# MiloszKrajewski/K4os.Compression.LZ4

Hardware: AMD Instinct MI355X
Metric: GiB/s encode+decode on batched 64 KiB blocks; bit-exact vs C# ref (higher is better)
Workload: dtype u8

## Files before the change

k4os/compression/lz4_amd/csrc/k4lz4_capi.hip:

```cpp
#include <hip/hip_runtime.h>
#include <stdint.h>
#include <stdio.h>
#include <stdlib.h>
#include <string.h>
#include <algorithm>
#include <atomic>
#include <memory>
#include <new>
#include <condition_variable>
#include <functional>
#include <mutex>
#include <string>
#include <thread>
#include <chrono>
#include <vector>

#include "../../../../include/k4lz4.h"
#include "k4lz4_decode.hpp"
#include "k4lz4_encode_fast.hpp"
#include "k4lz4_parse.hpp"
#include "k4lz4_pickle.hpp"
#include "k4lz4_segments.hpp"
#include "k4lz4_encode_hc.hpp"
#include "k4lz4_fast_chain.hpp"
#include "k4lz4_frame.hpp"
#include "k4lz4_frame_read.hpp"
#include "k4lz4_legacy.hpp"
#include "k4lz4_frame_write.hpp"
#include "k4lz4_frame_reader.hpp"
#include "k4lz4_frame_feed.hpp"
#include "k4lz4_legacy_stream.hpp"
#include "k4lz4_legacy_feed.hpp"
#include "k4lz4_chain_decoder.hpp"
#include "k4lz4_xxh32.hpp"
#include "k4lz4_selftest.hpp"

constexpr int MAX_PARTS = 8;

struct k4lz4_ctx {
    int device = -1;
    std::string error;
    hipStream_t stream = nullptr;
    int accel = 1;
    unsigned long long *prof = nullptr;
    bool prof_pair = false;
    bool prof_stamp = false;
    uint8_t *d_src = nullptr; size_t d_src_cap = 0;
    uint8_t *d_dst = nullptr; size_t d_dst_cap = 0;
    uint8_t *d_meta = nullptr; size_t d_meta_cap = 0;
    uint8_t *h_stage = nullptr; size_t h_stage_cap = 0;
    uint8_t *d_sched = nullptr; size_t d_sched_cap = 0;
    int cu_count = 256;
    uint8_t *d_dict = nullptr; size_t d_dict_cap = 0;
    uint8_t *d_gtab = nullptr; size_t d_gtab_cap = 0;
    hipStream_t aux = nullptr;
    hipStream_t aux2 = nullptr;
    hipEvent_t ev_join2 = nullptr;
    uint8_t *d_seg = nullptr; size_t d_seg_cap = 0;
    uint8_t *d_seg_first = nullptr; size_t d_seg_first_cap = 0;
    bool use_segments = true;
    uint32_t seg_min = 1024u << 10, seg_target = 640u << 10, seg_warm = 384u << 10;
    uint32_t seg_target_max = 1408u << 10;
    uint32_t seg_spin_max = 0;
    uint32_t seg_div = 3500;
    hipEvent_t ev_fork = nullptr, ev_join = nullptr;
    uint8_t *d_hc_hash = nullptr; size_t d_hc_hash_cap = 0;
    uint8_t *d_hc_work = nullptr; size_t d_hc_work_cap = 0;
    uint8_t *d_hc_meta = nullptr; size_t d_hc_meta_cap = 0;
    uint8_t *d_pk_meta = nullptr; size_t d_pk_meta_cap = 0;
    int pickle_split_min = 512;
    hipEvent_t ev_busy = nullptr;
    hipStream_t last_stream = nullptr;
    bool busy = false;
    uint64_t hc_res_total = 0; uint32_t hc_res_longest = 0;
    uint8_t *h_in[2] = {nullptr, nullptr}; size_t h_in_cap[2] = {0, 0};
    uint8_t *h_out[2] = {nullptr, nullptr}; size_t h_out_cap[2] = {0, 0};
    hipEvent_t ev_in[2] = {nullptr, nullptr}, ev_out[2] = {nullptr, nullptr};
    uint8_t *d_pack = nullptr; size_t d_pack_cap = 0;
    hipStream_t copyq = nullptr;
    hipStream_t dlq = nullptr;
    hipEvent_t ev_up[MAX_PARTS] = {}, ev_len[MAX_PARTS] = {};
    uint8_t *h_len = nullptr; size_t h_len_cap = 0;
    struct Pool *pool = nullptr, *pool_dl = nullptr;
    bool pool_failed = false, pool_dl_failed = false;
    int stage_threads = 7;
    uint32_t *d_pace = nullptr;
    uint32_t *d_status = nullptr;
    int split_pct = -1;
    bool no_pair = false;
    int direct_span_pct = 200;
    bool no_direct = false;
    int lds_floor_per_cu = 8;
    int cost_pct = 48;
    int dec_parts = 4, dec_parts_direct = 8;
    int hop2_max_per_cu = 12;
    bool hc_cand_lds = true;
    int hc_cand_dynlds = 0;
    int hc_segs = 0;
    bool hc_chain_parts = true;
    int hc_mem_pct = 33;
    int pace_min_per_cu = 6;
    bool use_pace = true;
    bool prof_gtab = false;
    uint8_t *d_parse = nullptr; size_t d_parse_cap = 0;
    bool use_parse = true;
    bool parse_queue = false;
    bool hc_records = true;
    bool parse_seg = true;
    bool parse_big = true;
    bool parse_persist = true;
    bool parse_inline_emit = true;
    bool parse_migrate = true;
    bool parse_pcost = false;
    int parse_waves = 16;
    bool trace = false;
    std::vector<uint8_t> h_chain;
    uint8_t *d_chain = nullptr; size_t d_chain_cap = 0;
    hipEvent_t ev_chain = nullptr;
    uint8_t *d_fr = nullptr; size_t d_fr_cap = 0;
    uint8_t *d_fb = nullptr; size_t d_fb_cap = 0;
    uint8_t *d_lg = nullptr; size_t d_lg_cap = 0;
    uint8_t *d_frd = nullptr; size_t d_frd_cap = 0;
    uint8_t *d_lgr = nullptr; size_t d_lgr_cap = 0;
    uint8_t *d_lga = nullptr; size_t d_lga_cap = 0;
    std::vector<uint8_t> h_fw;
    uint8_t *d_fw = nullptr; size_t d_fw_cap = 0;
    hipEvent_t ev_fw = nullptr;
};

struct Pool {
    std::vector<std::thread> workers;
    std::mutex m;
    std::condition_variable cv_work, cv_done;
    std::function<void(int)> job;
    int parts = 0, next = 0, pending = 0;
    unsigned long long gen = 0;
    bool stop = false;
    explicit Pool(int nthreads)
    {
        for (int t = 0; t < nthreads; t++) workers.emplace_back([this] { run(); });
    }
    ~Pool()
    {
        { std::lock_guard<std::mutex> g(m); stop = true; }
        cv_work.notify_all();
// ... 8 lines not shown
            const int i = next++;
            lk.unlock();
            job(i);
            lk.lock();
            if (--pending == 0) cv_done.notify_all();
        }
    }
    void parallel(int nparts, const std::function<void(int)> &f)
    {
        if (nparts <= 1 || workers.empty()) { for (int i = 0; i < nparts; i++) f(i); return; }
        std::unique_lock<std::mutex> lk(m);
        job = f; parts = nparts; next = 0; pending = nparts; gen++;
        cv_work.notify_all();
        while (next < parts) {
            const int i = next++;
            lk.unlock();
            f(i);
            lk.lock();
            if (--pending == 0) cv_done.notify_all();
        }
        cv_done.wait(lk, [this] { return pending == 0; });
        parts = 0;
    }
};

namespace {

thread_local std::string tl_error;
thread_local int tl_status = K4LZ4_OK;

std::mutex g_err_mu;
int fail(k4lz4_ctx *ctx, int code, const std::string &msg)
{
    if (ctx) { std::lock_guard<std::mutex> g(g_err_mu); ctx->error = msg; }
    tl_error = msg;
    return code;
}

int hip_fail(k4lz4_ctx *ctx, hipError_t e, const char *what)
{
    char buf[256];
    snprintf(buf, sizeof buf, "%s: %s", what, hipGetErrorString(e));
    (void)hipGetLastError();
    return fail(ctx, K4LZ4_E_HIP, buf);
}

#define K4_HIP(ctx, call)                                                   \
    do {                                                                    \
        hipError_t e_ = (call);                                             \
        if (e_ != hipSuccess) return hip_fail(ctx, e_, #call);              \
    } while (0)

enum Kind { KIND_ENCODE, KIND_DECODE, KIND_PICKLE, KIND_UNPICKLE, KIND_WRAP };
enum Envelope { ENV_NONE, ENV_PICKLE, ENV_WRAP };
constexpr int FLAG_SEGMENTS_OK = 1 << 20;

std::atomic<int> g_enforce32{0};

int check_level(k4lz4_ctx *ctx, int level)
{
    (void)ctx; (void)level;
    return K4LZ4_OK;
}

int grow(k4lz4_ctx *ctx, uint8_t **p, size_t *cap, size_t need, bool pinned);

int take_device_status(k4lz4_ctx *ctx)
// ... 238 lines not shown
            const int64_t cnt = std::min<int64_t>(chunk_max, n - first);
            const size_t need_meta = (size_t)cnt * 16 + 64;
            if (need_meta > ctx->d_pk_meta_cap) K4_HIP(ctx, hipStreamSynchronize(stream));
            int rc = grow(ctx, &ctx->d_pk_meta, &ctx->d_pk_meta_cap, need_meta, false);
            if (rc != K4LZ4_OK) return rc;
            uint64_t *d_encoff = (uint64_t *)ctx->d_pk_meta;
            int32_t *d_enccap = (int32_t *)(d_encoff + cnt);
            int32_t *d_enclen = d_enccap + cnt;
            k4::BatchArgs a{};
            a.src = src; a.srcOff = srcOff + first; a.srcLen = srcLen + first; a.dst = dst; a.dstOff = dstOff + first;
            a.dstCap = dstCap + first; a.outLen = outLen + first; a.n = cnt; a.level = level; a.accel = 1;
            a.flags = flags | (g_enforce32.load(std::memory_order_relaxed) ? K4LZ4_FLAG_X32 : 0);
            const int seg_ok = kind == KIND_PICKLE || may_cut ? FLAG_SEGMENTS_OK : 0;
            if (kind == KIND_PICKLE) hipLaunchKernelGGL(k4::k4_pickle_prep_kernel, dim3((unsigned)((cnt + 255) / 256)), dim3(256), 0, stream, a, d_encoff, d_enccap);
            else hipLaunchKernelGGL(k4::k4_wrap_prep_kernel, dim3((unsigned)((cnt + 255) / 256)), dim3(256), 0, stream, a, d_encoff, d_enccap);
            rc = launch_inner(ctx, KIND_ENCODE, src, srcOff + first, srcLen + first, dst, d_encoff, d_enccap, d_enclen, cnt, level,
                              (flags & (K4LZ4_FLAG_NO_REORDER | K4LZ4_FLAG_X32)) | K4LZ4_FLAG_RAW_RETURN | seg_ok, stream, nullptr, hostLen ? hostLen + first : nullptr);
            if (rc != K4LZ4_OK) return rc;
            if (kind == KIND_PICKLE) hipLaunchKernelGGL(k4::k4_pickle_finish_kernel, dim3((unsigned)((cnt + k4::PICKLE_FINISH_WAVES_PER_WG - 1) / k4::PICKLE_FINISH_WAVES_PER_WG)), dim3(64 * k4::PICKLE_FINISH_WAVES_PER_WG), 0, stream, a, d_enclen);
            else hipLaunchKernelGGL(k4::k4_wrap_finish_kernel, dim3((unsigned)((cnt + k4::WRAP_FINISH_WAVES_PER_WG - 1) / k4::WRAP_FINISH_WAVES_PER_WG)), dim3(64 * k4::WRAP_FINISH_WAVES_PER_WG), 0, stream, a, d_enclen);
            K4_HIP(ctx, hipGetLastError());
        }
        return K4LZ4_OK;
    }
    const bool reorder = n > 1 &&
                         (encode_like ? !(flags & K4LZ4_FLAG_NO_REORDER)
                                      : ((flags & K4LZ4_FLAG_REORDER) != 0 ||
                                         (kind == KIND_UNPICKLE && n > 64 && !(flags & K4LZ4_FLAG_NO_REORDER))));
    uint32_t *d_cost = nullptr, *d_order = nullptr, *d_hist = nullptr;
    if (reorder) {
        const size_t cnt_max = (size_t)std::min<int64_t>(chunk_max, n);
        const size_t hist_words = std::max<size_t>(2 * (size_t)k4::PCOST_BUCKETS, 2 * (size_t)k4::COST_BUCKETS + 16);
        const size_t need = cnt_max * 8 + hist_words * 4 + 64;
        if (need > ctx->d_sched_cap) K4_HIP(ctx, hipStreamSynchronize(stream));
        int rc = grow(ctx, &ctx->d_sched, &ctx->d_sched_cap, need, false);
        if (rc != K4LZ4_OK) return rc;
        d_hist = (uint32_t *)ctx->d_sched;
        d_cost = d_hist + hist_words;
        d_order = d_cost + cnt_max;
    }
    for (int64_t first = 0; first < n; first += chunk_max) {
        const int64_t cnt = std::min<int64_t>(chunk_max, n - first);
        k4::BatchArgs a{};
        a.src = src; a.srcOff = srcOff + first; a.srcLen = srcLen + first;
        a.dst = dst; a.dstOff = dstOff + first; a.dstCap = dstCap + first;
        a.outLen = outLen + first; a.n = cnt; a.level = level; a.accel = ctx->accel;
        a.flags = flags | (g_enforce32.load(std::memory_order_relaxed) ? K4LZ4_FLAG_X32 : 0);
        const bool hop2 = cnt <= (int64_t)ctx->hop2_max_per_cu * (int64_t)ctx->cu_count;
        a.prof = ctx->prof ? ctx->prof + k4::PROF_STRIDE * first : nullptr;
        a.status = ctx->d_status;
        if (((kind == KIND_ENCODE && !parse_path) || (K4_DEC_PACE && (kind == KIND_DECODE || kind == KIND_UNPICKLE))) && ctx->use_pace && ctx->d_pace && cnt > (int64_t)ctx->pace_min_per_cu * (int64_t)ctx->cu_count) {
            a.pace = ctx->d_pace;
            K4_HIP(ctx, hipMemsetAsync(a.pace, 0, k4::PACE_BYTES, stream));
        }
        k4::SegArgs sg{};
        bool seg = false;
        if (kind == KIND_ENCODE && (flags & (FLAG_SEGMENTS_OK | K4LZ4_FLAG_SEGMENTS)) && ctx->use_segments && !a.prof && !(flags & K4LZ4_FLAG_ALLOW_COPY)) {
            static_assert(k4::SEG_HDR_DWORDS * 4 == 256, "seg_first_of finds the header in front of the items");
            size_t max_items = (size_t)k4::SEG_MAX_ITEMS;
            if (hostLen) {
                size_t bound = 0;
                for (int64_t i = 0; i < cnt && bound < max_items; i++) {
                    const int32_t u = hostLen[first + i];
                    if (u > 0 && (uint32_t)u >= ctx->seg_min) bound += ((size_t)u + ctx->seg_target - 1) / ctx->seg_target;
                }
                max_items = std::min(max_items, std::max<size_t>(bound, 2));
            }
// ... 3 lines not shown
            if (total > ctx->d_seg_cap || (size_t)cnt * 4 > ctx->d_seg_first_cap) {
                K4_HIP(ctx, hipStreamSynchronize(stream));
                K4_HIP(ctx, hipStreamSynchronize(ctx->aux2));
            }
            int rc = grow(ctx, &ctx->d_seg, &ctx->d_seg_cap, total, false);
            if (rc == K4LZ4_OK) rc = grow(ctx, &ctx->d_seg_first, &ctx->d_seg_first_cap, (size_t)cnt * 4, false);
            if (rc != K4LZ4_OK) return rc;
            sg.hdr = (k4::SegHdr *)ctx->d_seg; sg.items = (k4::SegItem *)(ctx->d_seg + o_items); sg.work = (uint32_t *)(ctx->d_seg + o_work);
            sg.blocks = (uint32_t *)(ctx->d_seg + o_blocks); sg.snaps = (uint32_t *)(ctx->d_seg + o_snaps); sg.tables = (uint32_t *)(ctx->d_seg + o_tables);
            sg.first = (int32_t *)ctx->d_seg_first;
            sg.seg_min = ctx->seg_min; sg.seg_target = ctx->seg_target; sg.seg_warm = ctx->seg_warm; sg.seg_div = ctx->seg_div; sg.seg_target_max = ctx->seg_target_max; sg.spin_max = ctx->seg_spin_max; sg.max_items = (uint32_t)max_items;
            hipLaunchKernelGGL(k4::k4_seg_plan_kernel, dim3(1), dim3(256), 0, stream, a, sg);
            a.seg_first = sg.first; a.seg_items = sg.items; a.seg_snaps = sg.snaps;
            seg = true;
        }
        auto segments_start = [&]() -> int {
            if (!seg) return K4LZ4_OK;
            K4_HIP(ctx, hipEventRecord(ctx->ev_fork, stream));
            K4_HIP(ctx, hipStreamWaitEvent(ctx->aux2, ctx->ev_fork, 0));
            hipLaunchKernelGGL(k4::k4_encode_seg_kernel, dim3((unsigned)((sg.max_items + k4::ENCODE_WAVES_PER_WG - 1) / k4::ENCODE_WAVES_PER_WG)), dim3(64 * k4::ENCODE_WAVES_PER_WG), 0, ctx->aux2, a, sg);
            K4_HIP(ctx, hipEventRecord(ctx->ev_join2, ctx->aux2));
            return K4LZ4_OK;
        };
        auto segments_join = [&]() -> int {
            if (!seg) return K4LZ4_OK;
            K4_HIP(ctx, hipStreamWaitEvent(stream, ctx->ev_join2, 0));
            hipLaunchKernelGGL(k4::k4_seg_join_kernel, dim3((unsigned)std::min<int64_t>(k4::SEG_MAX_BLOCKS, cnt)), dim3(64), 0, stream, a, sg);
            return K4LZ4_OK;
        };
        if (dd && dd->dict) {
            a.dict = dd->dict; a.dictOff = dd->off + first; a.dictLen = dd->len + first;
            a.dictMode = dd->mode ? dd->mode + first : nullptr;
        }
        if (reorder && parse_path && kind == KIND_ENCODE && ctx->parse_pcost) {
            a.cost = d_cost; a.hist = d_hist; a.order_out = d_order;
            K4_HIP(ctx, hipMemsetAsync(d_hist, 0, 2 * k4::PCOST_BUCKETS * 4, stream));
            hipLaunchKernelGGL(k4::k4_pcost_kernel, dim3((unsigned)((cnt + k4::PCOST_WAVES_PER_WG - 1) / k4::PCOST_WAVES_PER_WG)), dim3(64 * k4::PCOST_WAVES_PER_WG), 0, stream, a);
            hipLaunchKernelGGL(k4::k4_porder_kernel, dim3((unsigned)((cnt + 255) / 256)), dim3(256), 0, stream, a);
            a.order = d_order;
        }
        else if (reorder) {
            a.cost = d_cost; a.hist = d_hist; a.order_out = d_order;
            K4_HIP(ctx, hipMemsetAsync(d_hist, 0, (2 * k4::COST_BUCKETS + 16) * 4, stream));
            hipLaunchKernelGGL(k4::k4_cost_kernel, dim3((unsigned)cnt), dim3(64), 0, stream, a, encode_like ? 0 : 1,
                               kind == KIND_ENCODE && parse_path ? k4::COST_SAMPLE_PARSE : k4::COST_SAMPLE);
            const bool two_kernels = kind == KIND_ENCODE && !a.prof && cnt > 512 && !(flags & K4LZ4_FLAG_NO_SPLIT) &&
                                     cnt > 8 * (int64_t)ctx->cu_count && ctx->split_pct <= 0;
            k4::BatchArgs ao = a;
            ao.first = two_kernels ? (uint32_t)ctx->cost_pct : 0u;
            ao.total = (uint32_t)((int64_t)ctx->lds_floor_per_cu * (int64_t)ctx->cu_count);
            hipLaunchKernelGGL(k4::k4_order_kernel, dim3((unsigned)((cnt + 255) / 256)), dim3(256), 0, stream, ao, (uint32_t)lds_share(ctx, cnt));
            a.order = d_order;
            if (two_kernels) a.split = d_hist + 2 * k4::COST_BUCKETS;
        }
        const unsigned wg4 = (unsigned)((cnt + k4::DECODE_WAVES_PER_WG - 1) / k4::DECODE_WAVES_PER_WG);
        bool parse_here = kind == KIND_ENCODE && (parse_path || (parse_seg_path && (a.order || cnt == 1)));
        const bool big_ok = ctx->parse_big && ctx->parse_inline_emit;
        bool any_small = true, any_big = big_ok;
        if (parse_here && hostLen) {
            any_small = false; any_big = false;
            for (int64_t i = 0; i < cnt && !(any_small && (any_big || !big_ok)); i++) {
                const int32_t len = hostLen[first + i];
                if (len >= (int32_t)k4::PARSE_MIN_LEN && len < k4::LIMIT_64K) any_small = true;
                else if (len >= k4::LIMIT_64K && big_ok) any_big = true;
            }
            parse_here = any_small || any_big;
        }
        int64_t waves = 0, nwg = 0, nwg_seg = 0;
        const bool seg_two_step = seg && parse_here && parse_seg_path;
        bool queue = false, slot_recs = false;
        size_t o_meta = 0, o_gtab = 0;
        if (parse_here) {
            waves = std::max<int64_t>(1, std::min<int64_t>(ctx->parse_waves, (cnt + ctx->cu_count - 1) / ctx->cu_count));
            queue = (ctx->parse_queue || parse_persistent || parse_seg_path) && a.order && cnt > waves * (int64_t)ctx->cu_count;
            nwg = queue ? (int64_t)ctx->cu_count : (cnt + waves - 1) / waves;
            if (seg_two_step) nwg_seg = std::min<int64_t>(ctx->cu_count, (cnt + (int64_t)sg.max_items + k4::PARSE_MAX_WAVES - 1) / k4::PARSE_MAX_WAVES);
            slot_recs = ctx->parse_inline_emit;
            const size_t rec_slots = slot_recs ? std::max((size_t)nwg * (size_t)waves, (size_t)nwg_seg * k4::PARSE_MAX_WAVES) : (size_t)cnt;
            o_meta = rec_slots * k4::PARSE_REC_STRIDE * sizeof(uint2); o_gtab = (o_meta + (size_t)cnt * 8 + 64 + 255) & ~(size_t)255;
            const size_t need = o_gtab + std::max(waves > k4::PARSE_LDS_TABLES ? (size_t)nwg * k4::PARSE_MAX_WAVES * 16384 : 0, (size_t)nwg_seg * k4::PARSE_MAX_WAVES * 16384);
            if (need > ctx->d_parse_cap) K4_HIP(ctx, hipStreamSynchronize(stream));
            const int rcp = grow(ctx, &ctx->d_parse, &ctx->d_parse_cap, need, false);
            if (rcp != K4LZ4_OK) { std::lock_guard<std::mutex> g(g_err_mu); ctx->error.clear(); parse_here = false; }
        }
        if (parse_here) {
            k4::ParseArgs pa{};
            pa.recs = (uint2 *)ctx->d_parse; pa.meta = (uint32_t *)(ctx->d_parse + o_meta); pa.gtab = (uint32_t *)(ctx->d_parse + o_gtab);
            pa.nwg = (uint32_t)nwg;
            pa.inline_emit = ctx->parse_inline_emit ? 1u : 0u;
            pa.slot_recs = slot_recs ? 1u : 0u;
            pa.migrate = ctx->parse_migrate ? 1u : 0u;
            pa.big = any_big ? 1u : 0u;
            K4_HIP(ctx, hipMemsetAsync(pa.meta + 2 * cnt, 0, 32, stream));
            if (queue) pa.queue = pa.meta + 2 * cnt;
            pa.nbig = pa.meta + 2 * cnt + 3;
            hipLaunchKernelGGL(k4::k4_parse_kernel, dim3((unsigned)nwg), dim3((unsigned)(64 * waves)), 0, stream, a, pa);
            if (seg_two_step) {
                k4::ParseArgs pb = pa;
                pb.queue = pa.meta + 2 * cnt + 4;
                pb.nwg = (uint32_t)nwg_seg;
                hipLaunchKernelGGL(k4::k4_parse_seg_kernel, dim3((unsigned)nwg_seg), dim3(64 * k4::PARSE_MAX_WAVES), 0, stream, a, pb, sg);
            } else if (any_big) {
                k4::ParseArgs pb = pa;
                if (queue) pb.queue = pa.queue + 4;
                hipLaunchKernelGGL(k4::k4_parse_big_kernel, dim3((unsigned)nwg), dim3((unsigned)(64 * waves)), 0, stream, a, pb);
            }
            if (!pa.inline_emit)
                hipLaunchKernelGGL(k4::k4_emit_kernel, dim3((unsigned)((cnt + k4::EMIT_WAVES_PER_WG - 1) / k4::EMIT_WAVES_PER_WG)), dim3(64 * k4::EMIT_WAVES_PER_WG), 0, stream, a, pa);
            bool rest = true;
            if (hostLen) {
                rest = false;
                for (int64_t i = 0; i < cnt && !rest; i++) rest = hostLen[first + i] < (int32_t)k4::PARSE_MIN_LEN || (hostLen[first + i] >= k4::LIMIT_64K && !any_big);
            }
            if (rest)
                hipLaunchKernelGGL(k4::k4_encode_fast_rest_kernel, dim3((unsigned)((cnt + k4::ENCODE_WAVES_PER_WG - 1) / k4::ENCODE_WAVES_PER_WG)), dim3(64 * k4::ENCODE_WAVES_PER_WG), 0, stream, a, pa);
            if (seg_two_step)
                hipLaunchKernelGGL(k4::k4_seg_join_kernel, dim3((unsigned)std::min<int64_t>(k4::SEG_MAX_BLOCKS, cnt)), dim3(64), 0, stream, a, sg);
            if (flags & K4LZ4_FLAG_ALLOW_COPY)
                hipLaunchKernelGGL(k4::k4_allow_copy_kernel, dim3((unsigned)((cnt + 3) / 4)), dim3(256), 0, stream, a);
            K4_HIP(ctx, hipGetLastError());
            continue;
        }
        switch (kind) {
        case KIND_ENCODE:
            if (a.prof && !ctx->prof_stamp) {
                if (ctx->prof_gtab) {
                    if ((size_t)cnt * 16384 > ctx->d_gtab_cap) {
                        K4_HIP(ctx, hipStreamSynchronize(ctx->aux));
                        int rc2 = grow(ctx, &ctx->d_gtab, &ctx->d_gtab_cap, (size_t)cnt * 16384, false);
                        if (rc2 != K4LZ4_OK) return rc2;
                    }
                    a.gtab = (uint32_t *)ctx->d_gtab;
                }
                hipLaunchKernelGGL(k4::k4_encode_fast_prof_kernel, dim3((unsigned)cnt), dim3(64), 0, stream, a);
            }
            else if (reorder && cnt > 512 && !(flags & K4LZ4_FLAG_NO_SPLIT)) {
                const int64_t lds_slots = 8 * (int64_t)ctx->cu_count;
                const int64_t n_lds = lds_share(ctx, cnt);
                const int64_t n_g = cnt - (a.split ? std::min<int64_t>(cnt, (int64_t)ctx->lds_floor_per_cu * (int64_t)ctx->cu_count) : n_lds);
                const int64_t gchunk = 8192;
                if (n_g > 0 && (size_t)std::min(n_g, gchunk) * 16384 > ctx->d_gtab_cap) {
                    K4_HIP(ctx, hipStreamSynchronize(ctx->aux));
                    int rc2 = grow(ctx, &ctx->d_gtab, &ctx->d_gtab_cap, (size_t)std::min(n_g, gchunk) * 16384, false);
                    if (rc2 != K4LZ4_OK) return rc2;
                }
                { const int rcs = segments_start(); if (rcs != K4LZ4_OK) return rcs; }
                K4_HIP(ctx, hipEventRecord(ctx->ev_fork, stream));
                K4_HIP(ctx, hipStreamWaitEvent(ctx->aux, ctx->ev_fork, 0));
                for (int64_t g0 = 0; g0 < n_g; g0 += gchunk) {
                    k4::BatchArgs ag = a;
                    ag.first = (uint32_t)((a.split ? 0 : n_lds) + g0);
                    ag.total = (uint32_t)cnt;
                    ag.gtab = (uint32_t *)ctx->d_gtab;
                    ag.n = std::min(gchunk, n_g - g0);
                    if (seg) hipLaunchKernelGGL(k4::k4_encode_fast_gtab_seg_kernel, dim3((unsigned)((ag.n + k4::ENCODE_WAVES_PER_WG - 1) / k4::ENCODE_WAVES_PER_WG)),
// ... 1113 lines not shown
    if (const char *pct = getenv("K4LZ4_SPLIT_PCT")) { const int v = atoi(pct); ctx->split_pct = v < 1 ? 1 : (v > 100 ? 100 : v); }
    ctx->no_pair = getenv("K4LZ4_NO_PAIR") != nullptr;
    ctx->prof_gtab = getenv("K4LZ4_PROF_GTAB") != nullptr;
    ctx->use_pace = getenv("K4LZ4_NO_PACE") == nullptr;
    if (const char *e = getenv("K4LZ4_PACE_MIN")) ctx->pace_min_per_cu = std::max(0, atoi(e));
    if (const char *e = getenv("K4LZ4_DIRECT_SPAN_PCT")) ctx->direct_span_pct = std::max(100, atoi(e));
    if (const char *e = getenv("K4LZ4_NO_DIRECT")) ctx->no_direct = atoi(e) != 0;
    if (const char *e = getenv("K4LZ4_LDS_FLOOR")) ctx->lds_floor_per_cu = std::max(0, std::min(8, atoi(e)));
    if (const char *e = getenv("K4LZ4_COST_PCT")) ctx->cost_pct = std::max(1, std::min(99, atoi(e)));
    if (const char *e = getenv("K4LZ4_DEC_PARTS")) ctx->dec_parts = std::max(2, std::min(MAX_PARTS, atoi(e)));
    if (const char *e = getenv("K4LZ4_DEC_PARTS_DIRECT")) ctx->dec_parts_direct = std::max(2, std::min(MAX_PARTS, atoi(e)));
    if (const char *e = getenv("K4LZ4_HOP2_MAX")) ctx->hop2_max_per_cu = std::max(0, atoi(e));
    ctx->hc_chain_parts = getenv("K4LZ4_HC_CHAIN_OLD") == nullptr;
    ctx->hc_cand_lds = getenv("K4LZ4_HC_CAND_MEM") == nullptr;
    if (const char *e = getenv("K4LZ4_HC_CAND_DYNLDS")) ctx->hc_cand_dynlds = std::max(0, std::min(65536, atoi(e)));
    if (const char *e = getenv("K4LZ4_HC_SEGS")) { const int v = atoi(e); ctx->hc_segs = v >= 4 ? 4 : (v >= 2 ? 2 : (v == 1 ? 1 : 0)); }
    if (const char *e = getenv("K4LZ4_HC_MEM_PCT")) ctx->hc_mem_pct = std::max(0, std::min(100, atoi(e)));
    ctx->use_segments = getenv("K4LZ4_NO_SEGMENTS") == nullptr;
    if (const char *e = getenv("K4LZ4_SEG_MIN")) ctx->seg_min = (uint32_t)std::max(65536 + 4096, atoi(e));
    if (const char *e = getenv("K4LZ4_SEG_TARGET")) ctx->seg_target = ctx->seg_target_max = (uint32_t)std::max(8192, atoi(e));
    if (const char *e = getenv("K4LZ4_SEG_TARGET_MAX")) ctx->seg_target_max = (uint32_t)std::max(8192, atoi(e));
    if (const char *e = getenv("K4LZ4_SEG_WARM")) ctx->seg_warm = (uint32_t)std::max(0, atoi(e));
    if (const char *e = getenv("K4LZ4_SEG_SPIN_MAX")) ctx->seg_spin_max = (uint32_t)std::max(0, atoi(e));
    if (const char *e = getenv("K4LZ4_SEG_DIV")) ctx->seg_div = (uint32_t)std::max(0, atoi(e));
    if (const char *e = getenv("K4LZ4_PICKLE_SPLIT_MIN")) ctx->pickle_split_min = std::max(0, atoi(e));
    if (const char *e = getenv("K4LZ4_STAGE_THREADS")) ctx->stage_threads = std::max(0, std::min(63, atoi(e) - 1));
    ctx->use_parse = getenv("K4LZ4_NO_PARSE") == nullptr;
    ctx->parse_queue = getenv("K4LZ4_PARSE_QUEUE") != nullptr;
    ctx->parse_persist = getenv("K4LZ4_NO_PERSIST") == nullptr;
    ctx->parse_big = getenv("K4LZ4_NO_PARSE_BIG") == nullptr;
    ctx->parse_seg = getenv("K4LZ4_NO_PARSE_SEG") == nullptr;
    ctx->hc_records = getenv("K4LZ4_NO_HC_RECORDS") == nullptr;
    ctx->parse_pcost = getenv("K4LZ4_PCOST") != nullptr;
    ctx->parse_migrate = getenv("K4LZ4_NO_MIGRATE") == nullptr;
    ctx->parse_inline_emit = getenv("K4LZ4_NO_INLINE_EMIT") == nullptr;
    if (const char *e = getenv("K4LZ4_PARSE_WAVES")) ctx->parse_waves = std::max(1, std::min(k4::PARSE_MAX_WAVES, atoi(e)));
    ctx->trace = getenv("K4LZ4_TRACE") != nullptr;
    if (e != hipSuccess) { delete ctx; return hip_fail(nullptr, e, "hipStreamCreate"); }
    *out = ctx;
    return K4LZ4_OK;
}

void k4lz4_ctx_destroy(k4lz4_ctx *ctx)
{
    if (!ctx) return;
    (void)hipSetDevice(ctx->device);
    if (ctx->stream) { (void)hipStreamSynchronize(ctx->stream); (void)hipStreamDestroy(ctx->stream); }
    if (ctx->aux) { (void)hipStreamSynchronize(ctx->aux); (void)hipStreamDestroy(ctx->aux); }
    if (ctx->aux2) { (void)hipStreamSynchronize(ctx->aux2); (void)hipStreamDestroy(ctx->aux2); }
    if (ctx->ev_join2) (void)hipEventDestroy(ctx->ev_join2);
    if (ctx->d_seg) (void)hipFree(ctx->d_seg);
    if (ctx->d_seg_first) (void)hipFree(ctx->d_seg_first);
    if (ctx->ev_fork) (void)hipEventDestroy(ctx->ev_fork);
    if (ctx->ev_join) (void)hipEventDestroy(ctx->ev_join);
    if (ctx->ev_busy) (void)hipEventDestroy(ctx->ev_busy);
    for (int b = 0; b < 2; b++) {
        if (ctx->ev_in[b]) (void)hipEventDestroy(ctx->ev_in[b]);
        if (ctx->ev_out[b]) (void)hipEventDestroy(ctx->ev_out[b]);
        if (ctx->h_in[b]) (void)hipHostFree(ctx->h_in[b]);
        if (ctx->h_out[b]) (void)hipHostFree(ctx->h_out[b]);
    }
    if (ctx->d_pack) (void)hipFree(ctx->d_pack);
    if (ctx->h_len) (void)hipHostFree(ctx->h_len);
    for (int b = 0; b < MAX_PARTS; b++) {
        if (ctx->ev_up[b]) (void)hipEventDestroy(ctx->ev_up[b]);
        if (ctx->ev_len[b]) (void)hipEventDestroy(ctx->ev_len[b]);
// ... 1874 lines not shown
```

k4os/compression/lz4_amd/csrc/k4lz4_encode_fast.hpp:

```cpp
#pragma once
#include "k4lz4_common.hpp"

namespace k4 {

#ifndef K4_SEG_WAVES_MIN
#define K4_SEG_WAVES_MIN 5
#endif
#ifndef K4_GTAB_DUTY
#define K4_GTAB_DUTY 3
#endif
#ifndef K4_PACE
#define K4_PACE 1
#endif

template <int TYPE> struct FastTable;

template <> struct FastTable<1> {
    uint16_t *t;
    __device__ __forceinline__ static uint32_t hash(const uint8_t *p) { return (ld32u(p) * 2654435761u) >> (32 - 13); }
    __device__ __forceinline__ static uint32_t hash_of(uint32_t seq, uint32_t) { return (seq * 2654435761u) >> (32 - 13); }
    __device__ __forceinline__ uint32_t get(uint32_t h) const { return t[h]; }
    __device__ __forceinline__ void put(uint32_t h, uint32_t pos) const { t[h] = (uint16_t)pos; }
    __device__ __forceinline__ uint32_t get_nt(uint32_t h) const
    {
// ... 817 lines not shown
{
    if (bkt < 4u) return bkt ? (unsigned long long)bkt * 4ull : 1ull;
    const uint32_t l = bkt >> 1;
    return ((bkt & 1u) ? 7ull : 5ull) << (l - 1u);
}

__global__ __launch_bounds__(256) void k4_order_kernel(BatchArgs a, uint32_t lds_max = 0xffffffffu)
{
    if (blockIdx.x == 0 && threadIdx.x == 0 && a.first != 0u) {
        unsigned long long all = 0;
        for (uint32_t k = 0; k < (uint32_t)COST_BUCKETS; k++) all += (unsigned long long)a.hist[k] * bucket_cost(k);
        const unsigned long long want = all / 100ull * (unsigned long long)a.first;
        unsigned long long have = 0, cnt = 0;
        for (int k = COST_BUCKETS - 1; k >= 0 && have < want; k--) {
            const unsigned long long c = a.hist[k], w = bucket_cost((uint32_t)k);
            if (have + c * w <= want) { have += c * w; cnt += c; }
            else { const unsigned long long part = (want - have + w - 1ull) / w; cnt += part; have = want; }
        }
        const unsigned long long floor_n = (unsigned long long)a.total < (unsigned long long)a.n ? (unsigned long long)a.total : (unsigned long long)a.n;
        if (cnt < floor_n) cnt = floor_n;
        if (cnt > (unsigned long long)a.n) cnt = (unsigned long long)a.n;
        if (cnt > (unsigned long long)lds_max) cnt = (unsigned long long)lds_max;
        a.hist[2 * COST_BUCKETS] = (uint32_t)cnt;
    }
    const long long b = (long long)blockIdx.x * 256 + threadIdx.x;
    if (b >= a.n) return;
    const uint32_t bkt = a.cost[b];
    uint32_t before = 0;
    for (uint32_t k = bkt + 1u; k < (uint32_t)COST_BUCKETS; k++) before += a.hist[k];
    const uint32_t pos = before + atomicAdd(&a.hist[COST_BUCKETS + bkt], 1u);
    a.order_out[pos] = (uint32_t)b;
}

constexpr int ENCODE_WAVES_PER_WG = 2;
struct SegFirst { SegRun run; uint32_t cap; bool cut; };
__device__ __forceinline__ SegFirst seg_first_of(const BatchArgs &a, long long b)
{
    SegFirst f;
    f.cut = false; f.cap = 0u;
    f.run.begin = 0u; f.run.emit_from = 0u; f.run.stop_at = SEG_NONE; f.run.snap_pub = nullptr; f.run.snap_chk = nullptr; f.run.resume = nullptr;
    f.run.cut = 0u; f.run.stop = 0u; f.run.state = 3u; f.run.spin_max = 0u; f.run.fix = nullptr;
    if (!a.seg_first) return f;
    const int32_t it = (int32_t)uni((uint32_t)a.seg_first[b]);
    if (it < 0) return f;
    const uint32_t *w = (const uint32_t *)a.seg_items + SEG_ITEM_WORDS * (uint32_t)it;
    f.cut = true;
    f.run.spin_max = uni(((const uint32_t *)a.seg_items)[-(int)SEG_HDR_DWORDS + 3]);
    f.run.stop_at = uni(w[4]);
    f.cap = f.run.stop_at;
    f.run.snap_chk = a.seg_snaps + (size_t)(it + 1) * SEG_SNAP_DWORDS;
    f.run.fix = a.seg_snaps + (size_t)uni(((const uint32_t *)a.seg_items)[-(int)SEG_HDR_DWORDS + 7]) * SEG_SNAP_DWORDS + 4096ull * (unsigned long long)it;
    return f;
}
__device__ __forceinline__ void seg_first_done(const BatchArgs &a, long long b, const SegFirst &f, int ret, int lane)
{
    if (!f.cut || lane != 0) return;
    uint32_t *w = (uint32_t *)a.seg_items + SEG_ITEM_WORDS * (uint32_t)a.seg_first[b];
    w[6] = f.run.cut; w[7] = f.run.stop; w[8] = ret > 0 ? f.run.state : 3u; w[9] = (uint32_t)ret;
}

template <bool MORE, bool SEG = false>
__device__ __forceinline__ void encode_fast_kernel_body(const BatchArgs &a, uint32_t (*tabs)[ENCODE_LDS_DWORDS])
{
    const int lane = lane_id();
    const uint32_t wave = uni(threadIdx.x >> 6);
    const long long slot = (long long)blockIdx.x * ENCODE_WAVES_PER_WG + (long long)wave;
// ... 95 lines not shown
```

k4os/compression/lz4_amd/csrc/k4lz4_parse.hpp:

```cpp
#pragma once
#include "k4lz4_encode_fast.hpp"
#include <type_traits>
#ifdef K4_PARSE_DEBUG
#include <stdio.h>
#include <stdlib.h>
#endif

namespace k4 {

#ifndef K4_PARSE_K
#define K4_PARSE_K 1
#endif

constexpr uint32_t PARSE_REC_STRIDE = 16448u;
static_assert(PARSE_REC_STRIDE >= ((uint32_t)LIMIT_64K - 1u - 6u) / 4u + 1u + 62u, "a block below LIMIT_64K has at most (LIMIT_64K - 1 - 6) / 4 sequences; a round adds at most 64 / 4 + 1");
constexpr uint32_t PARSE_MIN_LEN = 128u;
constexpr uint32_t PARSE_REST = 0xffffffffu;
constexpr uint32_t PARSE_BIG = 0xfffffffeu;
constexpr int PARSE_MAX_WAVES = 16;
constexpr int PARSE_LDS_TABLES = 9;
constexpr int PARSE_SEEN_DWORDS = 128;

constexpr int PARSE_LDS_DWORDS = 4096 * PARSE_LDS_TABLES + PARSE_SEEN_DWORDS * PARSE_MAX_WAVES + 4;

struct ParseArgs {
    uint2 *recs;
    uint32_t *meta;
    uint32_t *gtab;
    uint32_t nwg;
    uint32_t migrate;
    uint32_t inline_emit;
    uint32_t *nbig;
    uint32_t big;
    uint32_t slot_recs;
    uint32_t *queue;
};


template <int N> using ic = std::integral_constant<int, N>;
__device__ __forceinline__ unsigned long long uni64(unsigned long long v) { return ((unsigned long long)uni((uint32_t)(v >> 32)) << 32) | uni((uint32_t)v); }

__device__ __forceinline__ void shift16(uint32_t &w0, uint32_t &w1, uint32_t &w2, uint32_t &w3, uint32_t sh)
{
    if (sh == 0u) return;
    unsigned long long lo = ((unsigned long long)w1 << 32) | w0, hi = ((unsigned long long)w3 << 32) | w2;
    if (sh >= 16u) { lo = 0; hi = 0; }
    else if (sh >= 8u) { lo = sh == 8u ? hi : hi >> (8u * (sh - 8u)); hi = 0; }
    else { lo = (lo >> (8u * sh)) | (hi << (64u - 8u * sh)); hi >>= 8u * sh; }
    w0 = (uint32_t)lo; w1 = (uint32_t)(lo >> 32); w2 = (uint32_t)hi; w3 = (uint32_t)(hi >> 32);
}

__device__ __forceinline__ uint32_t ext12(uint32_t x0, uint32_t x1, uint32_t x2)
{
    const uint32_t t0 = min((uint32_t)(__ffs((int)x0) - 1), 32u);
    const uint32_t t1 = min((uint32_t)(__ffs((int)x1) - 1), 32u);
    const uint32_t t2 = min((uint32_t)(__ffs((int)x2) - 1), 32u);
    const uint32_t hi = t1 + (t1 == 32u ? t2 : 0u);
    return (t0 + (t0 == 32u ? hi : 0u)) >> 3;
}

__device__ __forceinline__ uint32_t ext28(const uint32_t *x)
{
    uint32_t acc = min((uint32_t)(__ffs((int)x[6]) - 1), 32u);
#pragma unroll
    for (int i = 5; i >= 0; i--) {
        const uint32_t t = min((uint32_t)(__ffs((int)x[i]) - 1), 32u);
        acc = t + (t == 32u ? acc : 0u);
    }
// ... 919 lines not shown
    const uint32_t waves = blockDim.x >> 6;
    const uint32_t lds_tables = waves < (uint32_t)PARSE_LDS_TABLES ? waves : (uint32_t)PARSE_LDS_TABLES;
    uint32_t *seen = lds + 4096u * (uint32_t)PARSE_LDS_TABLES + (uint32_t)PARSE_SEEN_DWORDS * wave;
    const bool in_lds = wave < lds_tables;
    if (U32 && p.nbig && uni(*(volatile uint32_t *)p.nbig) == 0u) return;
    if (p.migrate) {
        if (threadIdx.x == 0) lds[PARSE_LDS_DWORDS - 1] = 0u;
        __syncthreads();
    }
    for (long long idx = (long long)wave * (long long)p.nwg + (long long)blockIdx.x;;) {
        if (p.queue) {
            uint32_t t = 0u;
            if (lane == 0) {
                t = atomicAdd(p.queue, 1u);
                if (t < (uint32_t)a.n) t = in_lds ? atomicAdd(p.queue + 1, 1u) : (uint32_t)a.n - 1u - atomicAdd(p.queue + 2, 1u);
                else t = 0xffffffffu;
            }
            t = uni(t);
            if (t == 0xffffffffu) {
                if (p.migrate && in_lds && lane == 0) atomicOr(lds + PARSE_LDS_DWORDS - 1, 1u << wave);
                return;
            }
            idx = (long long)t;
        }
        if (idx >= a.n) return;
        const long long b = a.order ? (long long)uni(a.order[idx]) : idx;
        const int src_len = a.srcLen[b];
        uint32_t *meta = p.meta + 2ull * (unsigned long long)b;
        const bool big = src_len >= LIMIT_64K && a.accel == 1;
        const bool mine = a.accel == 1 && (U32 ? big : (src_len >= (int)PARSE_MIN_LEN && src_len < LIMIT_64K));
        if (!mine) {
            if (!U32 && lane == 0) {
                meta[0] = (big && p.big) ? PARSE_BIG : PARSE_REST; meta[1] = 0u;
                if (big && p.big && p.nbig) atomicAdd(p.nbig, 1u);
            }
        } else {
            uint32_t n = 0u;
            const int ret = parse_one<K, TT, false>(a, p, lds, seen, in_lds, wave, waves, lane, b, a.src + a.srcOff[b], src_len, a.dst + a.dstOff[b], a.dstCap[b], nullptr, &n);
            if (lane == 0) {
                meta[0] = n; meta[1] = 0u;
                if (p.inline_emit) a.outLen[b] = codec_encode_result(src_len, ret, a.flags);
            }
        }
        if (!p.queue) return;
    }
}


__global__ __launch_bounds__(64 * PARSE_MAX_WAVES) void k4_parse_kernel(BatchArgs a, ParseArgs p)
{
    __shared__ __attribute__((aligned(16))) uint32_t lds[PARSE_LDS_DWORDS];
    parse_kernel_body<K4_PARSE_K>(a, p, lds);
}

__global__ __launch_bounds__(64 * PARSE_MAX_WAVES) void k4_parse_big_kernel(BatchArgs a, ParseArgs p)
{
    __shared__ __attribute__((aligned(16))) uint32_t lds[PARSE_LDS_DWORDS];
    if (a.flags & FLAG_X32) parse_kernel_body<1, 2>(a, p, lds);
    else parse_kernel_body<1, 0>(a, p, lds);
}


constexpr uint32_t PCOST_SAMPLE = 3072u;
constexpr int PCOST_BUCKETS = 512;
constexpr int PCOST_WAVES_PER_WG = 8;

__device__ __forceinline__ uint32_t pcost_bucket(unsigned long long cost)
// ... 185 lines not shown
    return (int)op;
}

__global__ __launch_bounds__(64 * EMIT_WAVES_PER_WG) void k4_emit_kernel(BatchArgs a, ParseArgs p)
{
    const int lane = lane_id();
    const long long b = (long long)blockIdx.x * EMIT_WAVES_PER_WG + (long long)uni(threadIdx.x >> 6);
    if (b >= a.n) return;
    const uint32_t nseq = uni(p.meta[2ull * (unsigned long long)b]);
    if (nseq == PARSE_REST || nseq == PARSE_BIG) return;
    const int src_len = a.srcLen[b];
    const int cap = a.dstCap[b];
    const int ret = emit_block(a.src + a.srcOff[b], (uint32_t)src_len, a.dst + a.dstOff[b], cap < 0 ? 0 : cap,
                               p.recs + (unsigned long long)b * PARSE_REC_STRIDE, nseq, lane);
    if (lane == 0) a.outLen[b] = codec_encode_result(src_len, ret, a.flags);
}

__global__ __launch_bounds__(64 * ENCODE_WAVES_PER_WG) void k4_encode_fast_rest_kernel(BatchArgs a, ParseArgs p)
{
    __shared__ __attribute__((aligned(16))) uint32_t tabs[ENCODE_WAVES_PER_WG][ENCODE_LDS_DWORDS];
    const int lane = lane_id();
    const uint32_t wave = uni(threadIdx.x >> 6);
    const long long b = (long long)blockIdx.x * ENCODE_WAVES_PER_WG + (long long)wave;
    if (b >= a.n) return;
    if (uni(p.meta[2ull * (unsigned long long)b]) != PARSE_REST) return;
    const int src_len = a.srcLen[b];
    const int cap = a.dstCap[b];
    int ret = 0;
    if (src_len > 0 || (a.flags & FLAG_RAW_RETURN))
        ret = compress_fast_block<true, false>(a.src + a.srcOff[b], src_len, a.dst + a.dstOff[b], cap < 0 ? 0 : cap, a.accel, tabs[wave], lane, nullptr, (a.flags & FLAG_X32) != 0, nullptr);
    if (lane == 0) a.outLen[b] = codec_encode_result(src_len, ret, a.flags);
}

}
```

Before: 60.96.

## Fuse parse big and rest fallback kernels; add optional fused cost+order prelude

Adds a leftover kernel, on by default, that runs the big-block parse pass and then encodes the remaining PARSE_REST blocks in the same launch, reusing the parse LDS for the per-wave hash tables. The parse kernel now counts rest blocks so the leftover kernel can skip work early, and the separate rest-encode launch is dropped. An opt-in prelude kernel fuses cost sampling, histogram and ordering with a last-block-done pattern, removing memsets and a launch. This trades launch overhead for fewer rest waves per workgroup and grid-stride serial processing in the fused kernel.

```diff
diff --git a/k4os/compression/lz4_amd/csrc/k4lz4_capi.hip b/k4os/compression/lz4_amd/csrc/k4lz4_capi.hip
--- a/k4os/compression/lz4_amd/csrc/k4lz4_capi.hip
+++ b/k4os/compression/lz4_amd/csrc/k4lz4_capi.hip
@@ -50,6 +50,7 @@
     uint8_t *d_meta = nullptr; size_t d_meta_cap = 0;
     uint8_t *h_stage = nullptr; size_t h_stage_cap = 0;
     uint8_t *d_sched = nullptr; size_t d_sched_cap = 0;
+    bool hist_zero = false;
     int cu_count = 256;
     uint8_t *d_dict = nullptr; size_t d_dict_cap = 0;
     uint8_t *d_gtab = nullptr; size_t d_gtab_cap = 0;
@@ -111,6 +112,8 @@
     bool parse_persist = true;
     bool parse_inline_emit = true;
     bool parse_migrate = true;
+    bool fused_prelude = false;
+    bool fused_leftover = true;
     bool parse_pcost = false;
     int parse_waves = 16;
     bool trace = false;
@@ -185,7 +188,7 @@
 std::mutex g_err_mu;
 int fail(k4lz4_ctx *ctx, int code, const std::string &msg)
 {
-    if (ctx) { std::lock_guard<std::mutex> g(g_err_mu); ctx->error = msg; }
+    if (ctx) { std::lock_guard<std::mutex> g(g_err_mu); ctx->error = msg; ctx->hist_zero = false; }
     tl_error = msg;
     return code;
 }
@@ -490,7 +493,7 @@
         const size_t cnt_max = (size_t)std::min<int64_t>(chunk_max, n);
         const size_t hist_words = std::max<size_t>(2 * (size_t)k4::PCOST_BUCKETS, 2 * (size_t)k4::COST_BUCKETS + 16);
         const size_t need = cnt_max * 8 + hist_words * 4 + 64;
-        if (need > ctx->d_sched_cap) K4_HIP(ctx, hipStreamSynchronize(stream));
+        if (need > ctx->d_sched_cap) { ctx->hist_zero = false; K4_HIP(ctx, hipStreamSynchronize(stream)); }
         int rc = grow(ctx, &ctx->d_sched, &ctx->d_sched_cap, need, false);
         if (rc != K4LZ4_OK) return rc;
         d_hist = (uint32_t *)ctx->d_sched;
@@ -560,8 +563,20 @@
             a.dict = dd->dict; a.dictOff = dd->off + first; a.dictLen = dd->len + first;
             a.dictMode = dd->mode ? dd->mode + first : nullptr;
         }
+        bool prelude_pending = false;
+        k4::BatchArgs ap{};
+        auto launch_prelude = [&](uint32_t *zero8) -> int {
+            if (!prelude_pending) return K4LZ4_OK;
+            prelude_pending = false;
+            if (!ctx->hist_zero) K4_HIP(ctx, hipMemsetAsync(d_hist, 0, (2 * k4::COST_BUCKETS + 16) * 4, stream));
+            hipLaunchKernelGGL(k4::k4_prelude_kernel, dim3((unsigned)((cnt + k4::PRELUDE_WAVES_PER_WG - 1) / k4::PRELUDE_WAVES_PER_WG)), dim3(64 * k4::PRELUDE_WAVES_PER_WG), 0, stream,
+                               ap, parse_path ? k4::COST_SAMPLE_PARSE : k4::COST_SAMPLE, (uint32_t)lds_share(ctx, cnt), zero8);
+            ctx->hist_zero = true;
+            return K4LZ4_OK;
+        };
         if (reorder && parse_path && kind == KIND_ENCODE && ctx->parse_pcost) {
             a.cost = d_cost; a.hist = d_hist; a.order_out = d_order;
+            ctx->hist_zero = false;
             K4_HIP(ctx, hipMemsetAsync(d_hist, 0, 2 * k4::PCOST_BUCKETS * 4, stream));
             hipLaunchKernelGGL(k4::k4_pcost_kernel, dim3((unsigned)((cnt + k4::PCOST_WAVES_PER_WG - 1) / k4::PCOST_WAVES_PER_WG)), dim3(64 * k4::PCOST_WAVES_PER_WG), 0, stream, a);
             hipLaunchKernelGGL(k4::k4_porder_kernel, dim3((unsigned)((cnt + 255) / 256)), dim3(256), 0, stream, a);
@@ -569,15 +584,20 @@
         }
         else if (reorder) {
             a.cost = d_cost; a.hist = d_hist; a.order_out = d_order;
-            K4_HIP(ctx, hipMemsetAsync(d_hist, 0, (2 * k4::COST_BUCKETS + 16) * 4, stream));
-            hipLaunchKernelGGL(k4::k4_cost_kernel, dim3((unsigned)cnt), dim3(64), 0, stream, a, encode_like ? 0 : 1,
-                               kind == KIND_ENCODE && parse_path ? k4::COST_SAMPLE_PARSE : k4::COST_SAMPLE);
+            prelude_pending = kind == KIND_ENCODE && (parse_path || parse_seg_path) && ctx->fused_prelude && cnt <= k4::PRELUDE_MAX_BLOCKS;
+            if (!prelude_pending) {
+                ctx->hist_zero = false;
+                K4_HIP(ctx, hipMemsetAsync(d_hist, 0, (2 * k4::COST_BUCKETS + 16) * 4, stream));
+                hipLaunchKernelGGL(k4::k4_cost_kernel, dim3((unsigned)cnt), dim3(64), 0, stream, a, encode_like ? 0 : 1,
+                                   kind == KIND_ENCODE && parse_path ? k4::COST_SAMPLE_PARSE : k4::COST_SAMPLE);
+            }
             const bool two_kernels = kind == KIND_ENCODE && !a.prof && cnt > 512 && !(flags & K4LZ4_FLAG_NO_SPLIT) &&
                                      cnt > 8 * (int64_t)ctx->cu_count && ctx->split_pct <= 0;
             k4::BatchArgs ao = a;
             ao.first = two_kernels ? (uint32_t)ctx->cost_pct : 0u;
             ao.total = (uint32_t)((int64_t)ctx->lds_floor_per_cu * (int64_t)ctx->cu_count);
-            hipLaunchKernelGGL(k4::k4_order_kernel, dim3((unsigned)((cnt + 255) / 256)), dim3(256), 0, stream, ao, (uint32_t)lds_share(ctx, cnt));
+            if (prelude_pending) ap = ao;
+            else hipLaunchKernelGGL(k4::k4_order_kernel, dim3((unsigned)((cnt + 255) / 256)), dim3(256), 0, stream, ao, (uint32_t)lds_share(ctx, cnt));
             a.order = d_order;
             if (two_kernels) a.split = d_hist + 2 * k4::COST_BUCKETS;
         }
@@ -619,9 +639,12 @@
             pa.slot_recs = slot_recs ? 1u : 0u;
             pa.migrate = ctx->parse_migrate ? 1u : 0u;
             pa.big = any_big ? 1u : 0u;
-            K4_HIP(ctx, hipMemsetAsync(pa.meta + 2 * cnt, 0, 32, stream));
+            if (prelude_pending) { const int rcq = launch_prelude(pa.meta + 2 * cnt); if (rcq != K4LZ4_OK) return rcq; }
+            else K4_HIP(ctx, hipMemsetAsync(pa.meta + 2 * cnt, 0, 32, stream));
             if (queue) pa.queue = pa.meta + 2 * cnt;
             pa.nbig = pa.meta + 2 * cnt + 3;
+            const bool leftover = !hostLen && any_big && !seg_two_step && ctx->fused_leftover;
+            if (leftover) pa.nrest = pa.meta + 2 * cnt + 7;
             hipLaunchKernelGGL(k4::k4_parse_kernel, dim3((unsigned)nwg), dim3((unsigned)(64 * waves)), 0, stream, a, pa);
             if (seg_two_step) {
                 k4::ParseArgs pb = pa;
@@ -631,11 +654,12 @@
             } else if (any_big) {
                 k4::ParseArgs pb = pa;
                 if (queue) pb.queue = pa.queue + 4;
-                hipLaunchKernelGGL(k4::k4_parse_big_kernel, dim3((unsigned)nwg), dim3((unsigned)(64 * waves)), 0, stream, a, pb);
+                if (leftover) hipLaunchKernelGGL(k4::k4_parse_leftover_kernel, dim3((unsigned)nwg), dim3((unsigned)(64 * waves)), 0, stream, a, pb);
+                else hipLaunchKernelGGL(k4::k4_parse_big_kernel, dim3((unsigned)nwg), dim3((unsigned)(64 * waves)), 0, stream, a, pb);
             }
             if (!pa.inline_emit)
                 hipLaunchKernelGGL(k4::k4_emit_kernel, dim3((unsigned)((cnt + k4::EMIT_WAVES_PER_WG - 1) / k4::EMIT_WAVES_PER_WG)), dim3(64 * k4::EMIT_WAVES_PER_WG), 0, stream, a, pa);
-            bool rest = true;
+            bool rest = !leftover;
             if (hostLen) {
                 rest = false;
                 for (int64_t i = 0; i < cnt && !rest; i++) rest = hostLen[first + i] < (int32_t)k4::PARSE_MIN_LEN || (hostLen[first + i] >= k4::LIMIT_64K && !any_big);
@@ -649,6 +673,7 @@
             K4_HIP(ctx, hipGetLastError());
             continue;
         }
+        { const int rcq = launch_prelude(nullptr); if (rcq != K4LZ4_OK) return rcq; }
         switch (kind) {
         case KIND_ENCODE:
             if (a.prof && !ctx->prof_stamp) {
@@ -1828,6 +1853,8 @@
     ctx->parse_seg = getenv("K4LZ4_NO_PARSE_SEG") == nullptr;
     ctx->hc_records = getenv("K4LZ4_NO_HC_RECORDS") == nullptr;
     ctx->parse_pcost = getenv("K4LZ4_PCOST") != nullptr;
+    ctx->fused_prelude = getenv("K4LZ4_FUSED_PRELUDE") != nullptr;
+    ctx->fused_leftover = getenv("K4LZ4_NO_FUSED_LEFTOVER") == nullptr;
     ctx->parse_migrate = getenv("K4LZ4_NO_MIGRATE") == nullptr;
     ctx->parse_inline_emit = getenv("K4LZ4_NO_INLINE_EMIT") == nullptr;
     if (const char *e = getenv("K4LZ4_PARSE_WAVES")) ctx->parse_waves = std::max(1, std::min(k4::PARSE_MAX_WAVES, atoi(e)));
diff --git a/k4os/compression/lz4_amd/csrc/k4lz4_encode_fast.hpp b/k4os/compression/lz4_amd/csrc/k4lz4_encode_fast.hpp
--- a/k4os/compression/lz4_amd/csrc/k4lz4_encode_fast.hpp
+++ b/k4os/compression/lz4_amd/csrc/k4lz4_encode_fast.hpp
@@ -873,6 +873,86 @@
     a.order_out[pos] = (uint32_t)b;
 }
 
+constexpr int PRELUDE_WAVES_PER_WG = 4;
+constexpr int PRELUDE_DONE_WORD = 2 * COST_BUCKETS + 1;
+constexpr long long PRELUDE_MAX_BLOCKS = 65536;
+
+#ifdef K4_HOST_EMU
+__device__ __forceinline__ uint32_t load_agent(const uint32_t *p) { return *(const volatile uint32_t *)p; }
+__device__ __forceinline__ void fence_agent() { __sync_synchronize(); }
+#else
+__device__ __forceinline__ uint32_t load_agent(const uint32_t *p) { return __hip_atomic_load(p, __ATOMIC_RELAXED, __HIP_MEMORY_SCOPE_AGENT); }
+__device__ __forceinline__ void fence_agent() { __threadfence(); }
+#endif
+
+__global__ __launch_bounds__(64 * PRELUDE_WAVES_PER_WG) void k4_prelude_kernel(BatchArgs a, int sample_bytes, uint32_t lds_max, uint32_t *zero8)
+{
+    __shared__ __attribute__((aligned(16))) uint32_t tab[PRELUDE_WAVES_PER_WG][ENCODE_LDS_DWORDS];
+    __shared__ uint32_t s_cnt[COST_BUCKETS], s_pos[COST_BUCKETS], s_last;
+    const int lane = lane_id();
+    const uint32_t wave = uni(threadIdx.x >> 6);
+    const long long b = (long long)blockIdx.x * PRELUDE_WAVES_PER_WG + (long long)wave;
+    if (b < a.n) {
+        const int src_len = a.srcLen[b];
+        unsigned long long cost = 0;
+        if (src_len > 0) {
+            if (src_len <= 64) {
+                cost = (unsigned long long)src_len;
+            } else {
+                const int sample = src_len < sample_bytes ? src_len : sample_bytes;
+                uint32_t nseq = 0;
+                (void)encode_fast_block<true>(a.src + a.srcOff[b], sample, nullptr, 0x7fffffff, 1u, tab[wave], lane, nullptr, true, &nseq);
+                cost = ((unsigned long long)(nseq * 8u + (uint32_t)sample / 16u) * (unsigned long long)src_len) / (unsigned long long)sample;
+            }
+        }
+        if (lane == 0) {
+            const uint32_t bkt = cost_bucket(cost);
+            a.cost[b] = bkt;
+            atomicAdd(&a.hist[bkt], 1u);
+            fence_agent();
+        }
+    }
+    __syncthreads();
+    if (threadIdx.x == 0) {
+        fence_agent();
+        s_last = atomicAdd(&a.hist[PRELUDE_DONE_WORD], 1u) == gridDim.x - 1u ? 1u : 0u;
+    }
+    __syncthreads();
+    if (!s_last) return;
+    fence_agent();
+    if (threadIdx.x < (uint32_t)COST_BUCKETS) s_cnt[threadIdx.x] = load_agent(&a.hist[threadIdx.x]);
+    __syncthreads();
+    if (threadIdx.x == 0) {
+        uint32_t acc = 0;
+        for (int k = COST_BUCKETS - 1; k >= 0; k--) { s_pos[k] = acc; acc += s_cnt[k]; }
+        if (a.first != 0u) {
+            unsigned long long all = 0;
+            for (uint32_t k = 0; k < (uint32_t)COST_BUCKETS; k++) all += (unsigned long long)s_cnt[k] * bucket_cost(k);
+            const unsigned long long want = all / 100ull * (unsigned long long)a.first;
+            unsigned long long have = 0, cnt = 0;
+            for (int k = COST_BUCKETS - 1; k >= 0 && have < want; k--) {
+                const unsigned long long c = s_cnt[k], w = bucket_cost((uint32_t)k);
+                if (have + c * w <= want) { have += c * w; cnt += c; }
+                else { const unsigned long long part = (want - have + w - 1ull) / w; cnt += part; have = want; }
+            }
+            const unsigned long long floor_n = (unsigned long long)a.total < (unsigned long long)a.n ? (unsigned long long)a.total : (unsigned long long)a.n;
+            if (cnt < floor_n) cnt = floor_n;
+            if (cnt > (unsigned long long)a.n) cnt = (unsigned long long)a.n;
+            if (cnt > (unsigned long long)lds_max) cnt = (unsigned long long)lds_max;
+            a.hist[2 * COST_BUCKETS] = (uint32_t)cnt;
+        }
+    }
+    __syncthreads();
+    for (long long i = (long long)threadIdx.x; i < a.n; i += 64 * PRELUDE_WAVES_PER_WG) {
+        const uint32_t bkt = load_agent(&a.cost[i]);
+        const uint32_t pos = atomicAdd(&s_pos[bkt < (uint32_t)COST_BUCKETS ? bkt : (uint32_t)COST_BUCKETS - 1u], 1u);
+        if ((long long)pos < a.n) a.order_out[pos] = (uint32_t)i;
+    }
+    if (threadIdx.x < (uint32_t)COST_BUCKETS) a.hist[threadIdx.x] = 0u;
+    if (threadIdx.x == 0) a.hist[PRELUDE_DONE_WORD] = 0u;
+    if (zero8 && threadIdx.x < 8u) zero8[threadIdx.x] = 0u;
+}
+
 constexpr int ENCODE_WAVES_PER_WG = 2;
 struct SegFirst { SegRun run; uint32_t cap; bool cut; };
 __device__ __forceinline__ SegFirst seg_first_of(const BatchArgs &a, long long b)
diff --git a/k4os/compression/lz4_amd/csrc/k4lz4_parse.hpp b/k4os/compression/lz4_amd/csrc/k4lz4_parse.hpp
--- a/k4os/compression/lz4_amd/csrc/k4lz4_parse.hpp
+++ b/k4os/compression/lz4_amd/csrc/k4lz4_parse.hpp
@@ -34,6 +34,7 @@
     uint32_t big;
     uint32_t slot_recs;
     uint32_t *queue;
+    uint32_t *nrest;
 };
 
 
@@ -1019,7 +1020,8 @@
         if (!mine) {
             if (!U32 && lane == 0) {
                 meta[0] = (big && p.big) ? PARSE_BIG : PARSE_REST; meta[1] = 0u;
-                if (big && p.big && p.nbig) atomicAdd(p.nbig, 1u);
+                if (big && p.big) { if (p.nbig) atomicAdd(p.nbig, 1u); }
+                else if (p.nrest) atomicAdd(p.nrest, 1u);
             }
         } else {
             uint32_t n = 0u;
@@ -1271,4 +1273,34 @@
     if (lane == 0) a.outLen[b] = codec_encode_result(src_len, ret, a.flags);
 }
 
-}
+constexpr int LEFTOVER_REST_WAVES = PARSE_LDS_DWORDS / ENCODE_LDS_DWORDS;
+static_assert(LEFTOVER_REST_WAVES >= 1 && LEFTOVER_REST_WAVES <= PARSE_MAX_WAVES, "the rest blocks' waves take their tables from the parse kernel's LDS");
+
+__global__ __launch_bounds__(64 * PARSE_MAX_WAVES) void k4_parse_leftover_kernel(BatchArgs a, ParseArgs p)
+{
+    __shared__ __attribute__((aligned(16))) uint32_t lds[PARSE_LDS_DWORDS];
+    const uint32_t nbig = uni(*(volatile uint32_t *)p.nbig), nrest = uni(*(volatile uint32_t *)p.nrest);
+    if ((nbig | nrest) == 0u) return;
+    if (nbig != 0u) {
+        if (a.flags & FLAG_X32) parse_kernel_body<1, 2>(a, p, lds);
+        else parse_kernel_body<1, 0>(a, p, lds);
+    }
+    if (nrest == 0u) return;
+    __syncthreads();
+    const int lane = lane_id();
+    const uint32_t wave = uni(threadIdx.x >> 6);
+    const uint32_t waves = blockDim.x >> 6;
+    const uint32_t rest_waves = waves < (uint32_t)LEFTOVER_REST_WAVES ? waves : (uint32_t)LEFTOVER_REST_WAVES;
+    if (wave >= rest_waves) return;
+    for (long long b = (long long)blockIdx.x * rest_waves + (long long)wave; b < a.n; b += (long long)gridDim.x * rest_waves) {
+        if (uni(p.meta[2ull * (unsigned long long)b]) != PARSE_REST) continue;
+        const int src_len = a.srcLen[b];
+        const int cap = a.dstCap[b];
+        int ret = 0;
+        if (src_len > 0 || (a.flags & FLAG_RAW_RETURN))
+            ret = compress_fast_block<true, false>(a.src + a.srcOff[b], src_len, a.dst + a.dstOff[b], cap < 0 ? 0 : cap, a.accel, lds + (uint32_t)ENCODE_LDS_DWORDS * wave, lane, nullptr, (a.flags & FLAG_X32) != 0, nullptr);
+        if (lane == 0) a.outLen[b] = codec_encode_result(src_len, ret, a.flags);
+    }
+}
+
+}
```

Result: no change. 61.55 (median of 6 runs) (+1.0%).
